# urw7rs/diffusion-models-made-easy

Hardware: AMD Instinct MI355X
Metric: denoising steps/sec + training images/sec, DDPM UNet CIFAR10 32×32 @1/2/4/8 GPU (higher is better)
Workload: dtype bf16; 1 GPU; DDPM T=1000 sampling, CIFAR10 32x32, default UNet (32,416,643 params, random init), batch 128 per GPU, t.shape=(1,); global_batch=128, parallelism=dp1 (independent chains per GPU, no data-path collective)

## Files before the change

diffusion-models-made-easy_amd/_lib.py:

```python

from __future__ import annotations

import ctypes as C
import os
import subprocess
import threading

_HERE = os.path.dirname(os.path.abspath(__file__))
LIB_PATH = os.environ.get("DMME_LIB_PATH") or os.path.join(_HERE, "libdmme_hip.so")
CSRC = os.path.join(_HERE, "csrc")

F16R32 = 4
F32, BF16, BF16X3, F16 = 0, 1, 2, 3
CHAIN_DDPM, CHAIN_DDIM, CHAIN_IDDPM, CHAIN_DDPM_GUIDED, CHAIN_DDIM_GUIDED, CHAIN_GDDIM = 0, 1, 2, 3, 4, 5
CHAIN_DDPM_CFG, CHAIN_GDDIM_CFG = 6, 7
CHAIN_DPMPP, CHAIN_DPMPP_CFG = 8, 9
CHAIN_REPAINT = 10
ARCH_DDPM, ARCH_IDDPM, ARCH_CLASSIFIER, ARCH_DDPM_COND = 0, 1, 2, 3
DTYPES = {"fp32": F32, "float32": F32, "32": F32, "bf16": BF16, "bfloat16": BF16, "16": BF16, "bf16-mixed": BF16, "16-mixed": BF16,
          "bf16x3": BF16X3, "fp16": F16, "float16": F16, "half": F16, "fp16r32": F16R32}

_lock = threading.Lock()
_lib = None

# ... 85 lines not shown
    "dmme_unet_pack_params_bwd": (_i, [_vp, _vp, _vp, _vp]),
    "dmme_unet_backward": (_i, [_vp, _vp, _vp, _vp, _vp, _i, _vp, _vp, _vp, _vp, _vp, _vp, _vp]),
    "dmme_unet_backward_buckets": (_i, [_vp, _vp, _vp, _vp, _vp, _i, _vp, _vp, _vp, _vp, _vp, _vp, _vp, BUCKET_FN, _vp]),
    "dmme_unet_backward_input": (_i, [_vp, _vp, _vp, _vp, _vp, _i, _vp, _vp, _vp, _vp, _vp, _vp]),
    "dmme_unet_plan_grad_buckets": (_i, [_vp, C.POINTER(_i64), C.POINTER(_i64), C.POINTER(_i), _i]),
    "dmme_unet_plan_bwd_summary": (_i, [_vp, C.c_char_p, _i]),
    "dmme_grad_norm": (_i, [_vp, _i64, _vp, _vp, _vp]),
    "dmme_adam_step": (_i, [_vp, _vp, _vp, _vp, _vp, _i64, _f, _f, _f, _f, _i, _vp, _f, _f, _f, _vp]),
    "dmme_amp_init": (_i, [_vp, _f, _vp]),
    "dmme_amp_scale": (_i, [_vp, _i64, _vp, _vp]),
    "dmme_adam_step_amp": (_i, [_vp, _vp, _vp, _vp, _vp, _i64, _f, _f, _f, _f, _vp, _f, _f, _f, _vp, _f, _f, _i, _vp]),
    "dmme_grad_pack_bf16": (_i, [_vp, _i64, _vp, _i64, _vp]),
    "dmme_shard_reduce_bf16": (_i, [_vp, _i, _i64, _f, _vp, _vp]),
    "dmme_grad_unpack_bf16": (_i, [_vp, _i64, _vp, _vp]),
    "dmme_unet_debug_read": (_i, [_vp, _vp, C.c_char_p, _vp, _i64, C.POINTER(_i64), _vp]),
    "dmme_unet_debug_read_grad": (_i, [_vp, _vp, C.c_char_p, _vp, _i64, C.POINTER(_i64), _vp]),
    "dmme_dropout_masks": (_i, [_vp, _u64, _u64, _vp, _vp]),
    "dmme_randn": (_i, [_vp, _i64, _u64, _u64, _vp]),
    "dmme_q_sample": (_i, [_vp, _vp, _vp, _vp, _vp, _i, _i64, _vp, _vp, _vp]),
    "dmme_ddpm_step": (_i, [_vp, _vp, _vp, _f, _f, _f, _i, _i64, _vp]),
    "dmme_ddim_step": (_i, [_vp, _vp, _f, _f, _i64, _vp]),
    "dmme_gddim_step": (_i, [_vp, _vp, _vp, _f, _f, _f, _i64, _vp]),
    "dmme_slerp": (_i, [_vp, _vp, _vp, _i, _i, _i64, _vp, _vp]),
    "dmme_chain_set": (_i, [_vp, _i64, _vp, _u64, _u64, _vp]),
    "dmme_chain_update": (_i, [_i, _vp, _vp, _vp, _vp, _vp, _i, _i64, _vp]),
    "dmme_chain_step": (_i, [_vp, _vp, _vp, _vp, _vp, _i, _vp, _vp, _vp, _vp]),
    "dmme_chain_update_gddim": (_i, [_vp, _vp, _vp, _vp, _vp, _vp, _i, _i64, _vp]),
    "dmme_log_softmax_grad": (_i, [_vp, _vp, _i, _i, _i, _f, _vp, _vp, _vp, _vp]),
    "dmme_chain_update_guided": (_i, [_i, _vp, _vp, _vp, _vp, _vp, _vp, _vp, _i, _i64, _vp]),
    "dmme_guided_chain_step": (_i, [_vp, _vp, _vp, _vp, _vp, _vp, _vp, _vp, _vp, _vp, _vp, _vp, _vp, _vp, _vp, _i, _vp, _vp, _vp, _vp]),
    "dmme_mse_loss": (_i, [_vp, _vp, _i64, _vp, _vp, _f, _vp, _vp]),
    "dmme_image_batch": (_i, [_vp, _i64, _vp, _vp, _i, _i, _i, _i, _vp, _vp]),
    "dmme_grid_tile": (_i, [_vp, _i, _i, _i, _i, _i, _i, _i, _i, _i, _i, _i, _vp, _vp]),
    "dmme_iddpm_step": (_i, [_vp, _vp, _vp, _f, _f, _f, _f, _i, _i, _i64, _vp]),
    "dmme_iddpm_loss": (_i, [_vp, _vp, _vp, _vp, _vp, _vp, _i, _i64, _f, _f, _vp, _vp, _f, _vp, _vp]),
    "dmme_iddpm_loss_rows": (_i, [_vp, _vp, _vp, _vp, _vp, _vp, _i, _vp, _i, _i64, _f, _f, _vp, _vp, _vp, _f, _vp, _vp, _vp]),
    "dmme_iddpm_prior_rows": (_i, [_vp, _i, _i64, _f, _vp, _vp]),
    "dmme_tsampler_draw": (_i, [_vp, _vp, _i, _i, _f, _u64, _u64, _i, _vp, _vp, _vp, _vp]),
    "dmme_tsampler_update": (_i, [_vp, _vp, _i, _i, _vp, _vp, _i, _vp, _vp]),
    "dmme_conv2d": (_i, [C.POINTER(ConvDesc), _vp, _vp, _vp, _vp, _vp, _vp, _vp, _vp, _vp, _vp, _i, _vp, _vp]),
    "dmme_conv2d_res": (_i, [C.POINTER(ConvDesc), _vp, _vp, _vp, _vp, _vp, _vp, _vp, _vp, _vp, _i, _i, _vp, _vp, _vp, _vp]),
    "dmme_groupnorm_scale_shift": (_i, [_i, _vp, _vp, _i, _i, _i, _i, _i, _vp, _vp, _f, _vp, _vp, _vp, _i, _vp]),
    "dmme_attention": (_i, [_i, _vp, _i, _i, _i, _vp, _i, _vp]),
    "dmme_attention_proj": (_i, [_i, _vp, _i, _i, _i, _vp, _vp, _vp, _vp, _vp, _vp, _i, _vp]),
    "dmme_attention_heads": (_i, [_i, _vp, _i, _i, _i, _i, _vp, _i, _vp]),
    "dmme_nchw_to_nhwc": (_i, [_i, _vp, _i, _i, _i, _vp, _vp]),
    "dmme_nhwc_to_nchw": (_i, [_i, _vp, _i, _i, _i, _vp, _vp]),
    "dmme_pack_weight": (_i, [_i, _vp, _i, _i, _i, _vp, _vp]),
    "dmme_event_create": (_i, [C.POINTER(_vp)]),
    "dmme_event_record": (_i, [_vp, _vp]),
    "dmme_event_elapsed_ms": (_i, [_vp, _vp, C.POINTER(_f)]),
    "dmme_event_destroy": (_i, [_vp]),
    "dmme_debug_set_stamps": (_i, [_vp]),
    "dmme_debug_mfma_valu": (_i, [_i, _i, _i, _vp, _vp]),
    "dmme_debug_issue_probe": (_i, [_i, _i, _i, _i, _i, _vp, _vp, _vp]),
    "dmme_debug_l2_stream": (_i, [_vp, _i64, _i, _i, _i, _i, _vp, _vp]),
}


def lib():
    global _lib
    if _lib is not None:
        return _lib
    with _lock:
        if _lib is not None:
            return _lib
        if not os.path.exists(LIB_PATH):
            raise DmmeError(
                f"{LIB_PATH} is missing: the HIP extension is not built. Run `python -c 'import __graft_entry__ as g; g.build()'` "
                "(or `make -C diffusion-models-made-easy_amd/csrc`). There is no CPU fallback for the product path."
            )
        h = C.CDLL(LIB_PATH)
        for name, (res, args) in PROTOTYPES.items():
            fn = getattr(h, name)
            fn.restype = res
            fn.argtypes = args
        _lib = h
    return _lib


def check(rc: int, what: str = ""):
    if rc != 0:
        msg = lib().dmme_last_error().decode("utf-8", "replace")
        if rc == -2:
            raise NotImplementedError(f"{what}: {msg}")
        if rc == -1:
            raise ValueError(f"{what}: {msg}")
        raise DmmeError(f"{what} failed (status {rc}): {msg}")


def require_gpu():
    if lib().dmme_device_count() <= 0:
        raise DmmeError("libdmme_hip.so loaded but no HIP device is visible; the denoiser path only runs on an MI355X")


def dtype_code(precision) -> int:
    key = str(precision).lower()
    if key not in DTYPES:
        raise ValueError(f"unknown precision {precision!r}; use 'fp32', 'bf16', 'fp16' / 'fp16r32' (inference) or 'bf16x3'")
    return DTYPES[key]


def csrc_sha16() -> str:
    import glob
    import hashlib

# ... 19 lines not shown
```

diffusion-models-made-easy_amd/csrc/common.h:

```cpp
#pragma once

#include <hip/hip_runtime.h>
#include <stdint.h>

#include "dmme_hip.h"

namespace dmme {

void set_error(const char* fmt, ...) __attribute__((format(printf, 1, 2)));

int debug_route(const char* key, int dflt = 0);

#define DMME_CHECK_HIP(expr)                                                                          \
    do {                                                                                              \
        hipError_t e_ = (expr);                                                                       \
        if (e_ != hipSuccess) {                                                                       \
            ::dmme::set_error("%s failed: %s (%s:%d)", #expr, hipGetErrorString(e_), __FILE__, __LINE__); \
            return DMME_ERR_HIP;                                                                      \
        }                                                                                             \
    } while (0)

#define DMME_REQUIRE(cond, code, ...)        \
    do {                                     \
        if (!(cond)) {                       \
// ... 203 lines not shown
    CONV3X3_KW,
    CONV3X3_PIPE,
};
struct ConvRoute {
    int family;
    ConvTile tile;
    int BM, BN;
    int cand;
    int GT, UA;
    int NI, ring;
    int ksplit;
    int rseg;
    int vec;
    int stat_bn;
    int stat_px;
    int stat_tiles;
};
inline ConvRoute make_route(int family, int BM = 0, int BN = 0, int vec = 0) {
    ConvRoute r{};
    r.family = family;
    r.BM = r.stat_px = BM;
    r.BN = r.stat_bn = BN;
    r.vec = vec;
    return r;
}
ConvRoute conv_route(int dtype, const ConvArgs& a);
bool conv_thin_route(int dtype, const ConvArgs& a, ConvRoute& r);
bool conv1x1_split_route(int dtype, const ConvArgs& a, ConvRoute& r);
bool conv1x1_domain(int dtype, const ConvArgs& a);
bool conv1x1_as_route(int dtype, const ConvArgs& a, ConvRoute& r);
bool conv1x1_tiled_route(int dtype, const ConvArgs& a, ConvRoute& r);
bool conv3x3_split_route(int dtype, const ConvArgs& a, ConvRoute& r);
bool conv3x3_pipe_route(int dtype, const ConvArgs& a, ConvRoute& r);
bool conv3x3_ws_route(int dtype, const ConvArgs& a, ConvRoute& r);
bool conv3x3_kw_route(int dtype, const ConvArgs& a, ConvRoute& r);
bool conv_mfma_route(int dtype, const ConvArgs& a, ConvRoute& r);
void conv_generic_route(const ConvArgs& a, ConvRoute& r);
bool conv_mfma_supported(int dtype, const ConvArgs& a);
int launch_conv_generic(int dtype, const ConvArgs& a, hipStream_t s);
const char* conv_generic_kernel_name(const ConvArgs& a);
int launch_conv_mfma(const ConvRoute& r, int dtype, const ConvArgs& a, hipStream_t s);
int launch_conv_out_thin(const ConvArgs& a, hipStream_t s);
int launch_conv1x1(const ConvRoute& r, int dtype, const ConvArgs& a, hipStream_t s);
int launch_conv1x1_as(const ConvArgs& a, hipStream_t s);
int launch_conv3x3(const ConvRoute& r, int dtype, const ConvArgs& a, hipStream_t s);
int launch_conv_kw(int dtype, const ConvArgs& a, const ConvTile& g, int NI, int ring, int BM, int ksplit, hipStream_t s);
int launch_conv(int dtype, const ConvArgs& a, hipStream_t s, int force = 0);
int launch_conv(const ConvRoute& r, int dtype, const ConvArgs& a, hipStream_t s);
void conv_label(const ConvRoute& r, int dtype, const ConvArgs& a, char* buf, int cap);
bool conv_stats_query(int dtype, const ConvArgs& a, int cg, int* tiles, int* px);
bool conv_gn_in_query(int dtype, const ConvArgs& a);
bool conv1x1_tiled_gn_in_ok(const ConvArgs& a, const ConvRoute& r);
bool conv3x3_pipe_gn_in_ok(int dtype, const ConvArgs& a, const ConvRoute& r);
int conv_gn_direct_query(int dtype, const ConvArgs& a, const int* cg, int n);
int launch_gn_finalize_parts(const float* part1, int tiles1, int cnt1, int C1, const float* part2, int tiles2, int cnt2, int C2, int N, int groups,
                             const float* gamma, const float* beta, float eps, float* scale, float* shift, float* mean_rstd, const float* t_shift,
                             const float* t_scale, int t_ld, int nt, hipStream_t s);

int launch_gn_generic(int dtype, const void* src1, const void* src2, int N, int HW, int C1, int C2, int groups,
                      const float* gamma, const float* beta, float eps, float* scale, float* shift, float* mean_rstd,
                      hipStream_t s);
bool gn_fast_supported(int dtype, int N, int HW, int C1, int C2, int groups);
size_t gn_fast_scratch_floats(int N, int HW, int C, int groups);
int launch_gn_fast(int dtype, const void* src1, const void* src2, int N, int HW, int C1, int C2, int groups,
                   const float* gamma, const float* beta, float eps, float* scale, float* shift, float* mean_rstd,
                   float* partial, hipStream_t s, void* act = nullptr, int act_silu = 0, const float* dmask = nullptr);
bool gn_small_act_supported(int dtype, int HW, int C1, int C2, int groups);

int launch_attn_generic(int dtype, const void* qkv, int N, int S, int C, void* out, hipStream_t s);
int launch_attn_heads(int dtype, const void* qkv, int N, int S, int C, int heads, void* out, hipStream_t s);
int launch_attn_heads_bwd(int dtype, const void* qkv, const void* dO, int N, int S, int C, int heads, float* P, float* dS, void* dqkv, hipStream_t s);
int launch_gn_modulate(float* scale, float* shift, const float* t_shift, const float* t_scale, int ld, int nt, int N, int C, hipStream_t s);
bool attn_x3_supported(int N, int S, int C, int heads);
int launch_attn_x3(const void* qkv, int N, int S, int C, int heads, void* out, hipStream_t s);
bool attn_mfma_supported(int dtype, int N, int S, int C);
bool attn_full_takes(int S, int D);
int launch_attn_mfma(int dtype, const void* qkv, int N, int S, int C, void* out, float* lse, hipStream_t s);
bool attn_proj_fusable(int dtype, int N, int S, int C, int gn_cg, int gn_tiles);
int launch_attn_proj(int dtype, const void* qkv, int N, int S, int C, void* ctx, float* lse, const void* w, const float* bias, const void* res, void* dst,
                     float* gn_part, int gn_tiles, int gn_cg, hipStream_t s, long long* stamps = nullptr);
bool attn_heads_mfma_supported(int dtype, int N, int S, int C, int heads);
int launch_attn_heads_mfma(int dtype, const void* qkv, int N, int S, int C, int heads, void* out, float* lse, hipStream_t s);
int launch_attn_heads_bwd_mfma(int dtype, const void* qkv, const void* O, const void* dO, const float* lse, int N, int S, int C, int heads, void* P,
                               void* dS, void* dqkv, hipStream_t s);
bool attn_bwd_mfma_supported(int dtype, int N, int S, int C);
int launch_attn_bwd_mfma(int dtype, const void* qkv, const void* O, const void* dO, const float* lse, int N, int S, int C, void* P, void* dS,
                         void* dqkv, hipStream_t s);

constexpr unsigned kFwdMarkKeep = 0x4B454550u, kFwdMarkNograd = 0x4E4F4752u;
constexpr unsigned kErrNogradBackward = 0x80000000u;
int launch_time_sinusoid(const int64_t* t, int nt, const float* freqs, int half, float* out, hipStream_t s, unsigned* mark = nullptr,
                         unsigned mark_val = 0);
int launch_linear_wave(int dtype, const float* in, int nt, int K, const void* W, const float* bias, int Nout,
                       int out_silu, float* out, hipStream_t s);
int launch_label_cond(const float* z2, int nt, const float* E, const int64_t* labels, int B, int K, int emb, float* temb, float* zsave, int* status,
                      hipStream_t s);
int launch_label_grad(const float* dz2, const int64_t* labels, int B, int K, int emb, float* dE, hipStream_t s);

int launch_nchw_to_nhwc(int dtype, const float* src, int N, int C, int HW, void* dst, hipStream_t s, const unsigned* mark = nullptr,
                        unsigned* err = nullptr);
int launch_nhwc_to_nchw(int dtype, const void* src, int N, int C, int HW, float* dst, hipStream_t s);
int launch_pack_weight(int dtype, const float* src, int Cout, int Cin, int taps, void* dst, hipStream_t s);
int launch_cast_f32_to_16(int dtype, const float* src, int64_t numel, void* dst, hipStream_t s);

struct PackItem {
    int64_t src_off;
// ... 191 lines not shown
```

diffusion-models-made-easy_amd/csrc/conv_pipe.hip:

```cpp
#include <stdio.h>

#include "conv_common.h"

namespace dmme {



template <typename T, int BM, int BN, int GT, int PIPE_UA, bool ACC3 = false>
__global__ void __launch_bounds__(256, GT == 9 ? 1 : 2) conv3x3_pipe_kernel(ConvArgs a, ConvTile g, int shTW, int shTH, int ksplit) {
    constexpr int KC = Frag<T>::KC, EPV = Frag<T>::EPV;
    constexpr int MI = BM / 64, NI = BN / 64;
    constexpr int UB = BN / 32;
    extern __shared__ __attribute__((aligned(16))) char lds[];
#define PIPE_STAMP(K) do { if (a.stamps && blockIdx.x < 2 && blockIdx.y == 0 && threadIdx.x == 0) a.stamps[blockIdx.x * 8 + (K)] = (long long)wall_clock64(); } while (0)
    PIPE_STAMP(0);
    char* ldsA = lds;
    char* ldsB = lds + (size_t)g.a_rows * ROW_DATA;
    constexpr bool DMAB_OK = sizeof(T) == 2 && GT == 3 && BN == 64;
    constexpr int B_BYTES = GT * BN * ROW_DATA;
    const bool dmab = DMAB_OK && a.dma_b;
    int cur = 0;
    float* gni_par = reinterpret_cast<float*>(ldsB + (size_t)B_BYTES * (dmab ? 2 : 1));

    const int tid = threadIdx.x, lane = tid & 63, wave = tid >> 6;
// ... 203 lines not shown
                    __syncthreads();
                    store_A(nc0);
                }
                wait_vm_all();
                __syncthreads();
                cur ^= 1;
            } else {
                __syncthreads();
                if (more) {
                    store_B();
                    if (last_grp) store_A(nc0);
                }
                __syncthreads();
            }
        }
    }

    auto pix_of = [&](int m) -> int {
        const int tx = m & mTW, ty = (m >> shTW) & mTH, tn = m >> (shTW + shTH);
        const int n = n0 + tn;
        return n < a.N ? (n * a.Hout + oy0 + ty) * a.Wout + ox0 + tx : -1;
    };
    PIPE_STAMP(3);
    if (ksplit > 1) {
        float* part = a.splitk + (int64_t)blockIdx.y * a.N * a.Hout * a.Wout * a.Cout;
#pragma unroll
        for (int ni = 0; ni < NI; ++ni) {
            const int co = co0 + wn0 + ni * 32 + r;
            if (co >= a.Cout) continue;
#pragma unroll
            for (int mi = 0; mi < MI; ++mi)
#pragma unroll
                for (int j = 0; j < 16; ++j) {
                    const int opix = pix_of(wm0 + mi * 32 + (j & 3) + 8 * (j >> 2) + 4 * h);
                    if (opix >= 0) part[(int64_t)opix * a.Cout + co] = acc[mi][ni][j];
                }
        }
        PIPE_STAMP(4);
        return;
    }
    if constexpr (BM == 64) {
        if (a.n_gno > 0) {
            const bool add_trow = a.tproj && a.nt != 1 && g.TN > 1;
            conv_epilogue_stage<T, BN, MI, NI>(a, acc, co0, wn0, r, h, wm0, n0, reinterpret_cast<float*>(lds), !add_trow);
            __syncthreads();
            conv_epilogue_store_direct<T, BN>(a, co0, n0, a.Hout * a.Wout, pix_of, reinterpret_cast<float*>(lds), add_trow);
            PIPE_STAMP(4);
            return;
        }
    }
    conv_epilogue<T, BM, BN, MI, NI>(a, acc, co0, wn0, r, h, wm0, n0, g.TN, pix_of, reinterpret_cast<float*>(lds), ty_blk * g.tiles_x + tx_blk);
    PIPE_STAMP(4);
#undef PIPE_STAMP
}

template <typename T>
__global__ void __launch_bounds__(256) conv_splitk_finish_kernel(ConvArgs a, int ksplit, int64_t total4) {
    const int C4 = a.Cout / 4, hw = a.Hout * a.Wout;
    const int64_t slice = (int64_t)a.N * hw * a.Cout;
    for (int64_t q = blockIdx.x * (int64_t)blockDim.x + threadIdx.x; q < total4; q += (int64_t)gridDim.x * blockDim.x) {
        const int64_t p = q / C4;
        const int c = (int)(q - p * C4) * 4;
        float4 v = *reinterpret_cast<const float4*>(a.splitk + p * a.Cout + c);
        for (int z = 1; z < ksplit; ++z) {
            const float4 u = *reinterpret_cast<const float4*>(a.splitk + z * slice + p * a.Cout + c);
            v.x += u.x; v.y += u.y; v.z += u.z; v.w += u.w;
        }
        float f[4] = {v.x, v.y, v.z, v.w};
        const int n = (int)(p / hw);
#pragma unroll
        for (int j = 0; j < 4; ++j) {
            float fold = a.bias ? a.bias[c + j] : 0.f;
            if (a.tproj) fold += a.tproj[(int64_t)(a.nt == 1 ? 0 : n) * a.tproj_ld + c + j];
            f[j] += fold;
            if (a.res1) f[j] += to_f(((const T*)a.res1)[p * a.Cout + c + j]);
            ((T*)a.dst)[p * a.Cout + c + j] = from_f<T>(f[j]);
        }
    }
}
static int pipe_ksplit(const ConvArgs& a, const ConvTile& g, int pick, int KC) {
    if (a.has_gni) return 1;
    const bool off = (debug_route("no_splitk") != 0);
    if (off || !a.splitk || pick != 3 || a.stride != 1 || a.gn_part || a.n_gno || a.out_silu || a.out_nchw || a.res2 || a.Cout % 4) return 1;
    const int64_t wgs = (int64_t)g.tiles_m * g.tiles_n;
    if (wgs > 128) return 1;
    int ks = (a.C1 + a.C2) / KC;
    const int room = (int)(256 / wgs);
    if (ks > room) ks = room;
    if (ks > 4) ks = 4;
    const int64_t out = (int64_t)a.N * a.Hout * a.Wout * a.Cout;
    while (ks > 1 && ks * out > a.splitk_cap) --ks;
    return ks < 1 ? 1 : ks;
}

#ifndef WS_CDMA
#define WS_CDMA 1
#endif
#ifndef WS_HYB
#define WS_HYB 0
#endif
#ifndef WS_SCHED2
#define WS_SCHED2 1
#endif
#ifndef WS_TP_UNROLL
#define WS_TP_UNROLL 9
#endif
// ... 924 lines not shown
static int launch_ws2_split(const ConvRoute& r, const ConvArgs& a, hipStream_t s) {
    const ConvTile& gw = r.tile;
    static bool attr = false;
    if (!attr) {
        int rc0 = set_lds_limit(conv3x3_ws2_kernel<11, f16, 256, 1>, 160 * 1024);
        if (rc0 == DMME_OK) rc0 = set_lds_limit(conv3x3_ws2_kernel<11, f16, 256, 2>, 160 * 1024);
        if (rc0 != DMME_OK) return rc0;
        attr = true;
    }
    const int ntiles = gw.tiles_m * gw.tiles_n;
    const dim3 wgrid((unsigned)(ntiles < 256 ? ntiles : 256));
    if (a.mix == 2)
        hipLaunchKernelGGL((conv3x3_ws2_kernel<11, f16, 256, 2>), wgrid, dim3(512), ws2_lds(a, gw), s, a, gw, ilog2(gw.TW), ilog2(gw.TH), ntiles);
    else
        hipLaunchKernelGGL((conv3x3_ws2_kernel<11, f16, 256, 1>), wgrid, dim3(512), ws2_lds(a, gw), s, a, gw, ilog2(gw.TW), ilog2(gw.TH), ntiles);
    DMME_CHECK_LAUNCH();
    return DMME_OK;
}

template <typename T>
static int launch_ws_t(const ConvRoute& r, const ConvArgs& a, hipStream_t s) {
    const ConvTile& gw = r.tile;
    static bool ws_attr = false;
    if (!ws_attr) {
        int rc0 = set_lds_limit(conv3x3_ws2_kernel<11, T, 256>, 160 * 1024);
        if (rc0 == DMME_OK) rc0 = set_lds_limit(conv3x3_ws2_kernel<7, T, 128>, 160 * 1024);
        if (rc0 == DMME_OK) rc0 = set_lds_limit(conv3x3_ws2_kernel<11, T, 256, 0, true>, 160 * 1024);
        if (rc0 == DMME_OK) rc0 = set_lds_limit(conv3x3_ws2_kernel<7, T, 128, 0, true>, 160 * 1024);
        if (rc0 == DMME_OK) rc0 = set_lds_limit(conv3x3_ws2_kernel<11, T, 256, 0, false, true>, 160 * 1024);
        if (rc0 == DMME_OK) rc0 = set_lds_limit(conv3x3_ws2_kernel<11, T, 256, 0, true, true>, 160 * 1024);
        if (rc0 != DMME_OK) return rc0;
        ws_attr = true;
    }
    const int ntiles = gw.tiles_m * gw.tiles_n;
    const dim3 wgrid((unsigned)(ntiles < 256 ? ntiles : 256));
    const bool e16 = !a.res1 && !a.res2 && !debug_route("no_ws_e16");
    if (a.r_w) {
        if (r.BM == 128)
            hipLaunchKernelGGL((conv3x3_ws2_kernel<7, T, 128, 0, true>), wgrid, dim3(512), ws2_lds(a, gw), s, a, gw, ilog2(gw.TW), ilog2(gw.TH), ntiles);
        else if (e16)
            hipLaunchKernelGGL((conv3x3_ws2_kernel<11, T, 256, 0, true, true>), wgrid, dim3(512), ws2_lds(a, gw), s, a, gw, ilog2(gw.TW), ilog2(gw.TH), ntiles);
        else
            hipLaunchKernelGGL((conv3x3_ws2_kernel<11, T, 256, 0, true>), wgrid, dim3(512), ws2_lds(a, gw), s, a, gw, ilog2(gw.TW), ilog2(gw.TH), ntiles);
    } else if (r.BM == 128)
        hipLaunchKernelGGL((conv3x3_ws2_kernel<7, T, 128>), wgrid, dim3(512), ws2_lds(a, gw), s, a, gw, ilog2(gw.TW), ilog2(gw.TH), ntiles);
    else if (e16)
        hipLaunchKernelGGL((conv3x3_ws2_kernel<11, T, 256, 0, false, true>), wgrid, dim3(512), ws2_lds(a, gw), s, a, gw, ilog2(gw.TW), ilog2(gw.TH), ntiles);
    else
        hipLaunchKernelGGL((conv3x3_ws2_kernel<11, T, 256>), wgrid, dim3(512), ws2_lds(a, gw), s, a, gw, ilog2(gw.TW), ilog2(gw.TH), ntiles);
    DMME_CHECK_LAUNCH();
    return DMME_OK;
}

template <typename T, bool ACC3 = false>
static int launch_pipe_t(const ConvRoute& r, int dtype, const ConvArgs& a, hipStream_t s) {
    const ConvTile& g = r.tile;
    const int ksplit = r.ksplit;
    const dim3 grid((unsigned)(g.tiles_m * g.tiles_n), (unsigned)ksplit);
    ConvArgs ad = a;
    bool dma = false;
    const size_t lds = pipe_launch_lds(dtype, a, r, &dma);
    ad.dma_b = dma ? 1 : 0;
    const int shTW = ilog2(g.TW), shTH = ilog2(g.TH);
    static bool attr_done[5] = {false, false, false, false, false};
    int rc = DMME_OK;
#define DMME_PIPE_CASE(IDX, BM_, BN_, GT_, UA_, LIM)                                                                          \
    case IDX:                                                                                                                 \
        if (!attr_done[IDX]) {                                                                                                \
            rc = set_lds_limit(conv3x3_pipe_kernel<T, BM_, BN_, GT_, UA_, ACC3>, (LIM) * 1024);                               \
            attr_done[IDX] = rc == DMME_OK;                                                                                   \
        }                                                                                                                     \
        if (rc == DMME_OK) hipLaunchKernelGGL((conv3x3_pipe_kernel<T, BM_, BN_, GT_, UA_, ACC3>), grid, dim3(256), lds, s, ad, g, shTW, shTH, ksplit); \
        break;
    switch (r.cand) {
        DMME_PIPE_CASE(0, 128, 128, 3, 8, 80)
        DMME_PIPE_CASE(1, 128, 64, 3, 8, 80)
        DMME_PIPE_CASE(2, 64, 64, 3, 8, 80)
        DMME_PIPE_CASE(3, 64, 64, 9, 11, 128)
        DMME_PIPE_CASE(4, 64, 64, 3, 10, 80)
    }
#undef DMME_PIPE_CASE
    if (rc != DMME_OK) return rc;
    DMME_CHECK_LAUNCH();
    if (ksplit > 1) {
        const int64_t total4 = (int64_t)a.N * a.Hout * a.Wout * (a.Cout / 4);
        hipLaunchKernelGGL(conv_splitk_finish_kernel<T>, dim3((unsigned)((total4 + 255) / 256)), dim3(256), 0, s, a, ksplit, total4);
        DMME_CHECK_LAUNCH();
    }
    return DMME_OK;
}

int launch_conv3x3(const ConvRoute& r, int dtype, const ConvArgs& a, hipStream_t s) {
    switch (r.family) {
        case CONV3X3_SPLIT: return launch_ws2_split(r, a, s);
        case CONV3X3_WS: return dtype == DMME_F16 ? launch_ws_t<f16>(r, a, s) : launch_ws_t<bf16>(r, a, s);
        case CONV3X3_KW: return launch_conv_kw(dtype, a, r.tile, r.NI, r.ring, r.BM, r.ksplit, s);
        default: break;
    }
    if (dtype == DMME_BF16) return launch_pipe_t<bf16>(r, dtype, a, s);
    if (dtype == DMME_F16) return launch_pipe_t<f16>(r, dtype, a, s);
    return a.x3 ? launch_pipe_t<float, true>(r, dtype, a, s) : launch_pipe_t<float>(r, dtype, a, s);
}

}
```

diffusion-models-made-easy_amd/csrc/plan.hip:

```cpp
#include "plan.h"

#include <functional>
#include <map>
#include <mutex>

namespace dmme {

static thread_local char g_err[512] = "";
void set_error(const char* fmt, ...) {
    va_list ap;
    va_start(ap, fmt);
    vsnprintf(g_err, sizeof(g_err), fmt, ap);
    va_end(ap);
}

int debug_route(const char* key, int dflt) {
    const char* e = getenv("DMME_DEBUG_ROUTE");
    if (!e || !*e) return dflt;
    const size_t kl = strlen(key);
    for (const char* p = e; *p;) {
        const char* end = strchr(p, ',');
        const size_t len = end ? (size_t)(end - p) : strlen(p);
        if (len >= kl && !strncmp(p, key, kl) && (len == kl || p[kl] == '=')) return len == kl ? 1 : atoi(p + kl + 1);
        if (!end) break;
// ... 1738 lines not shown
    DMME_REQUIRE(eps && target && loss && scratch, DMME_ERR_INVALID, "mse_loss: null argument");
    return launch_mse(eps, target, numel, loss, d_eps, grad_scale, scratch, (hipStream_t)stream);
}

DMME_API int dmme_debug_issue_probe(int kind, int n_inner, int iters, int flags, int blocks, void* sink, const void* src, void* stream) {
    return launch_issue_probe(kind, n_inner, iters, flags, blocks, (long long*)sink, src, (hipStream_t)stream);
}
DMME_API int dmme_debug_mfma_valu(int mode, int iters, int blocks, void* sink, void* stream) {
    DMME_REQUIRE(sink && iters > 0 && blocks > 0, DMME_ERR_INVALID, "mfma_valu: bad argument");
    return launch_mfma_valu(mode, iters, blocks, (float*)sink, (hipStream_t)stream);
}
DMME_API int dmme_debug_l2_stream(const void* buf, int64_t bytes, int iters, int mode, int depth, int blocks, void* sink, void* stream) {
    return launch_l2_stream(buf, bytes, iters, mode, depth, blocks, (unsigned*)sink, (hipStream_t)stream);
}

static long long* g_stamps = nullptr;
DMME_API int dmme_debug_set_stamps(void* buf) {
    g_stamps = (long long*)buf;
    return DMME_OK;
}

DMME_API int dmme_conv2d(const dmme_conv_desc* d, const void* src1, const void* src2, const void* weight, const float* bias,
                const float* scale, const float* shift, const float* dmask, const float* tproj, const void* res1,
                const void* res2, int R1, void* dst, void* stream) {
    DMME_REQUIRE(d && src1 && weight && bias && dst, DMME_ERR_INVALID, "conv2d: null argument");
    DMME_REQUIRE(d->taps == 9 || d->taps == 1, DMME_ERR_INVALID, "conv2d: taps must be 1 or 9");
    DMME_REQUIRE(d->stride == 1 || d->stride == 2, DMME_ERR_INVALID, "conv2d: stride must be 1 or 2");
    ConvArgs a{};
    a.src1 = src1; a.src2 = src2; a.w = weight; a.bias = bias; a.scale = scale; a.shift = shift; a.dmask = dmask;
    a.tproj = d->nt > 0 ? tproj : nullptr;
    a.res1 = res1; a.res2 = res2; a.R1 = R1; a.dst = dst;
    a.N = d->N; a.Hin = d->Hin; a.Win = d->Win; a.C1 = d->C1; a.C2 = src2 ? d->C2 : 0;
    a.up = d->upsample; a.stride = d->stride; a.taps = d->taps;
    const int Hv = a.up ? 2 * a.Hin : a.Hin, Wv = a.up ? 2 * a.Win : a.Win;
    a.Hout = Hv / a.stride; a.Wout = Wv / a.stride; a.Cout = d->Cout;
    a.pro_silu = d->pro_silu; a.out_silu = d->out_silu; a.nt = d->nt; a.tproj_ld = d->tproj_ld;
    a.in_nchw = d->in_nchw; a.out_nchw = d->out_nchw;
    a.stamps = g_stamps;
    DMME_REQUIRE(d->dtype == DMME_F32 || d->dtype == DMME_BF16 || d->dtype == DMME_BF16X3 || d->dtype == DMME_F16 || d->dtype == DMME_F16R32, DMME_ERR_INVALID,
                 "conv2d: bad dtype %d", d->dtype);
    a.x3 = d->dtype == DMME_BF16X3;
    a.f16 = d->dtype == DMME_F16;
    if (d->dtype == DMME_F16R32) {
        a.mix = a.out_nchw ? 3 : a.taps == 1 ? 4 : 1;
        a.f16 = 1;
        const ConvRoute r = conv_route(DMME_F16, a);
        DMME_REQUIRE(r.family == (a.mix == 4 ? CONV1X1_SPLIT : a.mix == 3 ? CONV_THIN : CONV3X3_SPLIT), DMME_ERR_UNSUPPORTED, "conv2d(fp16r32): the %s does not take this shape",
                     a.mix == 4 ? "split-pass 1x1 kernel" : a.mix == 3 ? "thin output conv" : "split-pass 3x3 kernel");
        return launch_conv(r, DMME_F16, a, (hipStream_t)stream);
    }
    return launch_conv(a.x3 ? DMME_F32 : d->dtype, a, (hipStream_t)stream, d->force_generic);
}

DMME_API int dmme_conv2d_res(const dmme_conv_desc* d, const void* src1, const void* src2, const void* weight, const float* bias, const float* scale,
                             const float* shift, const float* dmask, const void* r_src1, const void* r_src2, int r_C1, int r_C2, const void* r_weight,
                             const float* r_bias, void* dst, void* stream) {
    DMME_REQUIRE(d && src1 && weight && bias && dst && r_src1 && r_weight && r_bias, DMME_ERR_INVALID, "conv2d_res: null argument");
    DMME_REQUIRE(d->dtype == DMME_BF16 || d->dtype == DMME_F16, DMME_ERR_UNSUPPORTED, "conv2d_res: 16-bit tensors only (dtype %d)", d->dtype);
    ConvArgs a{};
    a.src1 = src1; a.src2 = src2; a.w = weight; a.bias = bias; a.scale = scale; a.shift = shift; a.dmask = dmask; a.dst = dst;
    a.N = d->N; a.Hin = d->Hin; a.Win = d->Win; a.C1 = d->C1; a.C2 = src2 ? d->C2 : 0;
    a.up = d->upsample; a.stride = d->stride; a.taps = d->taps;
    a.Hout = a.Hin; a.Wout = a.Win; a.Cout = d->Cout;
    a.pro_silu = d->pro_silu; a.out_silu = d->out_silu;
    a.f16 = d->dtype == DMME_F16;
    a.stamps = g_stamps;
    a.r_src1 = r_src1; a.r_src2 = r_C2 > 0 ? r_src2 : nullptr; a.r_C1 = r_C1; a.r_C2 = r_C2 > 0 ? r_C2 : 0; a.r_w = r_weight; a.r_bias = r_bias;
    const ConvRoute r = conv_route(d->dtype, a);
    DMME_REQUIRE(a.taps == 9 && a.stride == 1 && !a.up && r.rseg, DMME_ERR_UNSUPPORTED,
                 "conv2d_res: the wave-specialised 3x3 kernel does not take this shape with a residual segment (%d+%d -> %d channels, %d+%d raw, %dx%dx%d)", a.C1, a.C2,
                 a.Cout, a.r_C1, a.r_C2, a.N, a.Hin, a.Win);
    return launch_conv(r, d->dtype, a, (hipStream_t)stream);
}

DMME_API int dmme_groupnorm_scale_shift(int dtype, const void* src1, const void* src2, int N, int HW, int C1, int C2, int groups,
                               const float* gamma, const float* beta, float eps, float* scale, float* shift,
                               float* partial_scratch, int force_generic, void* stream) {
    DMME_REQUIRE(src1 && gamma && beta && scale && shift, DMME_ERR_INVALID, "groupnorm: null argument");
    if (!src2) C2 = 0;
    DMME_REQUIRE(groups > 0 && (C1 + C2) % groups == 0, DMME_ERR_INVALID, "groupnorm: %d channels not divisible by %d groups",
                 C1 + C2, groups);
    if (!force_generic && partial_scratch && gn_fast_supported(dtype, N, HW, C1, C2, groups))
        return launch_gn_fast(dtype, src1, src2, N, HW, C1, C2, groups, gamma, beta, eps, scale, shift, nullptr,
                              partial_scratch, (hipStream_t)stream);
    return launch_gn_generic(dtype, src1, src2, N, HW, C1, C2, groups, gamma, beta, eps, scale, shift, nullptr,
                             (hipStream_t)stream);
}

DMME_API int dmme_attention(int dtype, const void* qkv, int N, int S, int C, void* out, int force_generic, void* stream) {
    DMME_REQUIRE(qkv && out && N > 0 && S > 0 && C > 0, DMME_ERR_INVALID, "attention: bad argument");
    if (dtype == DMME_BF16X3) {
        if (!force_generic && attn_x3_supported(N, S, C, 1)) return launch_attn_x3(qkv, N, S, C, 1, out, (hipStream_t)stream);
        dtype = DMME_F32;
    }
    if (!force_generic && attn_mfma_supported(dtype, N, S, C)) return launch_attn_mfma(dtype, qkv, N, S, C, out, nullptr, (hipStream_t)stream);
    return launch_attn_generic(dtype, qkv, N, S, C, out, (hipStream_t)stream);
}

DMME_API int dmme_attention_proj(int dtype, const void* qkv, int N, int S, int C, const void* w, const float* bias, const void* res, void* dst, void* ctx,
                                 float* gn_part, int gn_cg, void* stream) {
    DMME_REQUIRE(qkv && w && bias && res && dst && N > 0 && S > 0 && C > 0, DMME_ERR_INVALID, "attention_proj: bad argument");
    return launch_attn_proj(dtype, qkv, N, S, C, ctx, nullptr, w, bias, res, dst, gn_part, S / 32, gn_cg, (hipStream_t)stream, g_stamps);
}

DMME_API int dmme_attention_heads(int dtype, const void* qkv, int N, int S, int C, int heads, void* out, int force_generic, void* stream) {
    DMME_REQUIRE(qkv && out && N > 0 && S > 0 && C > 0 && heads > 0 && C % heads == 0, DMME_ERR_INVALID, "attention_heads: bad argument");
// ... 45 lines not shown
```

include/dmme_hip.h:

```cpp
#ifndef DMME_HIP_H
#define DMME_HIP_H

#include <stddef.h>
#include <stdint.h>

#if defined(DMME_BUILD)
#define DMME_API __attribute__((visibility("default")))
#else
#define DMME_API
#endif

#ifdef __cplusplus
extern "C" {
#endif

typedef enum {
    DMME_OK = 0,
    DMME_ERR_INVALID = -1,
    DMME_ERR_UNSUPPORTED = -2,
    DMME_ERR_HIP = -3,
    DMME_ERR_NOMEM = -4
} dmme_status;

typedef enum { DMME_F32 = 0, DMME_BF16 = 1, DMME_BF16X3 = 2, DMME_F16 = 3, DMME_F16R32 = 4 } dmme_dtype;
// ... 188 lines not shown


DMME_API int dmme_iddpm_loss_rows(const float* model_out, const float* x_t, const float* x_0, const float* target, const int64_t* t,
                                  const float* coef, int T, const float* weight, int B, int64_t chw, float w_simple, float w_vlb, float* loss,
                                  float* rows, float* d_out, float grad_scale, int* status, float* scratch, void* stream);

DMME_API int dmme_iddpm_prior_rows(const float* x_0, int B, int64_t chw, float alpha_bar_T, float* prior, void* stream);

DMME_API int dmme_tsampler_draw(const float* hist, const int* count, int T, int H, float uniform_prob, uint64_t philox_seed,
                                uint64_t philox_offset, int B, int64_t* t, float* weight, float* p, void* stream);

DMME_API int dmme_tsampler_update(float* hist, int* count, int T, int H, const int64_t* t, const float* L, int B, int* status, void* stream);

typedef struct {
    int dtype;
    int N, Hin, Win;
    int C1, C2;
    int upsample;
    int stride;
    int taps;
    int Cout;
    int pro_silu;
    int out_silu;
    int nt;
    int tproj_ld;
    int in_nchw;
    int out_nchw;
    int force_generic;
} dmme_conv_desc;

DMME_API int dmme_conv2d(const dmme_conv_desc* d, const void* src1, const void* src2, const void* weight,
                const float* bias, const float* scale, const float* shift, const float* dmask,
                const float* tproj, const void* res1, const void* res2, int R1, void* dst, void* stream);

DMME_API int dmme_conv2d_res(const dmme_conv_desc* d, const void* src1, const void* src2, const void* weight, const float* bias,
                const float* scale, const float* shift, const float* dmask, const void* r_src1, const void* r_src2, int r_C1,
                int r_C2, const void* r_weight, const float* r_bias, void* dst, void* stream);

DMME_API int dmme_groupnorm_scale_shift(int dtype, const void* src1, const void* src2, int N, int HW, int C1, int C2,
                               int groups, const float* gamma, const float* beta, float eps, float* scale,
                               float* shift, float* partial_scratch, int force_generic, void* stream);

DMME_API int dmme_attention(int dtype, const void* qkv, int N, int S, int C, void* out, int force_generic, void* stream);
DMME_API int dmme_attention_proj(int dtype, const void* qkv, int N, int S, int C, const void* w, const float* bias, const void* res,
                                 void* dst, void* ctx, float* gn_part, int gn_cg, void* stream);

DMME_API int dmme_attention_heads(int dtype, const void* qkv, int N, int S, int C, int heads, void* out, int force_generic, void* stream);

DMME_API int dmme_nchw_to_nhwc(int dtype, const float* src, int N, int C, int HW, void* dst, void* stream);
DMME_API int dmme_nhwc_to_nchw(int dtype, const void* src, int N, int C, int HW, float* dst, void* stream);
DMME_API int dmme_pack_weight(int dtype, const float* src, int Cout, int Cin, int taps, void* dst, void* stream);

DMME_API int dmme_debug_set_stamps(void* buf);

DMME_API int dmme_event_create(void** ev);
DMME_API int dmme_event_record(void* ev, void* stream);
DMME_API int dmme_event_elapsed_ms(void* start, void* stop, float* ms);
DMME_API int dmme_event_destroy(void* ev);

#ifdef __cplusplus
}
#endif
#endif
```

Baseline: 450.9 denoising steps/s (one step = UNet forward + DDPM update on a batch of 128), summed over GPUs.

## Add persistent ring-buffered 3x3 stride-2 conv kernel with in-loop DMA interleave

Adds a new kernel for 16-bit 3x3 stride-2 downsampling convolutions. It is persistent, with the grid capped at 256 blocks, and it prefetches the next tile's halo and filter slices into LDS while the current tile computes. The global-to-LDS DMA is spread across the MFMA sequence, with explicit vmcnt waits and double-buffered halo regions, and the four waves' partial accumulators are reduced through LDS before the shared epilogue. The aim is to hide load latency and launch tail on the small downsample convs in the UNet. In exchange it uses a large LDS footprint (one block per CU), adds cross-wave reduction overhead, and is only eligible for a narrow set of shapes.

Measured after the change: 453.0 denoising steps/s (one step = UNet forward + DDPM update on a batch of 128), summed over GPUs (median of 6 runs). About the same (+0.5%).

```diff
diff --git a/diffusion-models-made-easy_amd/_lib.py b/diffusion-models-made-easy_amd/_lib.py
--- a/diffusion-models-made-easy_amd/_lib.py
+++ b/diffusion-models-made-easy_amd/_lib.py
@@ -161,6 +161,7 @@
     "dmme_event_elapsed_ms": (_i, [_vp, _vp, C.POINTER(_f)]),
     "dmme_event_destroy": (_i, [_vp]),
     "dmme_debug_set_stamps": (_i, [_vp]),
+    "dmme_debug_conv_body": (_i, [C.POINTER(ConvDesc)]),
     "dmme_debug_mfma_valu": (_i, [_i, _i, _i, _vp, _vp]),
     "dmme_debug_issue_probe": (_i, [_i, _i, _i, _i, _i, _vp, _vp, _vp]),
     "dmme_debug_l2_stream": (_i, [_vp, _i64, _i, _i, _i, _i, _vp, _vp]),
diff --git a/diffusion-models-made-easy_amd/csrc/common.h b/diffusion-models-made-easy_amd/csrc/common.h
--- a/diffusion-models-made-easy_amd/csrc/common.h
+++ b/diffusion-models-made-easy_amd/csrc/common.h
@@ -279,6 +279,7 @@
 bool conv_gn_in_query(int dtype, const ConvArgs& a);
 bool conv1x1_tiled_gn_in_ok(const ConvArgs& a, const ConvRoute& r);
 bool conv3x3_pipe_gn_in_ok(int dtype, const ConvArgs& a, const ConvRoute& r);
+int conv3x3_pipe_body(int dtype, const ConvArgs& a, const ConvRoute& r);
 int conv_gn_direct_query(int dtype, const ConvArgs& a, const int* cg, int n);
 int launch_gn_finalize_parts(const float* part1, int tiles1, int cnt1, int C1, const float* part2, int tiles2, int cnt2, int C2, int N, int groups,
                              const float* gamma, const float* beta, float eps, float* scale, float* shift, float* mean_rstd, const float* t_shift,
diff --git a/diffusion-models-made-easy_amd/csrc/conv_pipe.hip b/diffusion-models-made-easy_amd/csrc/conv_pipe.hip
--- a/diffusion-models-made-easy_amd/csrc/conv_pipe.hip
+++ b/diffusion-models-made-easy_amd/csrc/conv_pipe.hip
@@ -279,6 +279,244 @@
     conv_epilogue<T, BM, BN, MI, NI>(a, acc, co0, wn0, r, h, wm0, n0, g.TN, pix_of, reinterpret_cast<float*>(lds), ty_blk * g.tiles_x + tx_blk);
     PIPE_STAMP(4);
 #undef PIPE_STAMP
+}
+
+constexpr int S2R_PASSES = 11, S2R_PA = 6, S2R_PB = S2R_PASSES - S2R_PA;
+constexpr int S2R_HROWS = 32 * S2R_PASSES;
+constexpr int S2R_HBYTES = S2R_HROWS * ROW_DATA;
+constexpr int S2R_FBYTES = 3 * 64 * ROW_DATA;
+constexpr int S2R_OFF_F = S2R_HBYTES, S2R_OFF_H1 = S2R_HBYTES + 3 * S2R_FBYTES;
+constexpr int S2R_LDS = 2 * S2R_HBYTES + 3 * S2R_FBYTES;
+constexpr int S2R_NF = 6;
+static_assert(S2R_LDS <= 160 * 1024 && S2R_FBYTES + S2R_HBYTES >= 4 * 4 * 16 * 64 * 4 && kDirectLds <= S2R_FBYTES + S2R_HBYTES, "s2ring: LDS plan");
+struct S2Tile { int n0, oy0, ox0, co0, ts; };
+static_assert(S2R_PA + S2R_NF + S2R_PB < 64, "vmcnt is a 6-bit counter");
+
+__device__ __forceinline__ void wait_vm_all_visible() {
+#if defined(__HIP_DEVICE_COMPILE__)
+    __builtin_amdgcn_s_waitcnt(0x0F70);
+    asm volatile("" ::: "memory");
+#endif
+}
+
+template <typename T>
+__global__ void __launch_bounds__(256, 1) conv3x3_s2ring_kernel(ConvArgs a, ConvTile g, int shTW, int shTH, int ntiles) {
+    constexpr int KC = 64, EPV = 8, BM = 64, BN = 64;
+    extern __shared__ __attribute__((aligned(16))) char lds[];
+#define S2R_STAMP(K) do { if (a.stamps && blockIdx.x < 2 && threadIdx.x == 0) { a.stamps[blockIdx.x * 8 + (K)] = (long long)wall_clock64(); wait_vm_all_visible(); } } while (0)
+    S2R_STAMP(0);
+    const int tid = threadIdx.x, lane = tid & 63, wave = __builtin_amdgcn_readfirstlane(tid >> 6);
+    const int r = lane & 31, h = lane >> 5;
+    const int cu = tid & 7, urow = tid >> 3;
+    const int Cin = a.C1, nchunks = Cin / KC;
+    const int mTW = (1 << shTW) - 1, mTH = (1 << shTH) - 1;
+    const int halo_px = g.HH * g.HWd;
+    const unsigned lds0 = (unsigned)__builtin_amdgcn_readfirstlane((int)(unsigned)(size_t)(lds_c*)lds) + (unsigned)(wave * 8 * ROW_DATA);
+    const unsigned src_piece = (unsigned)((cu ^ ((urow >> 1) & 7)) * EPV);
+    const char* wbase = (const char*)a.w;
+    const char* sbase = (const char*)a.src1;
+
+    unsigned a_off[S2R_PASSES];
+    unsigned okmask = 0;
+    unsigned bd_off[2];
+    auto set_tile = [&](int t) __attribute__((always_inline)) -> S2Tile {
+        const int tile_n = t % g.tiles_n, tile_m = t / g.tiles_n;
+        const int tx_blk = tile_m % g.tiles_x, ty_blk = (tile_m / g.tiles_x) % g.tiles_y;
+        S2Tile w;
+        w.n0 = (tile_m / (g.tiles_x * g.tiles_y)) * g.TN;
+        w.oy0 = ty_blk << shTH;
+        w.ox0 = tx_blk << shTW;
+        w.co0 = tile_n * BN;
+        w.ts = ty_blk * g.tiles_x + tx_blk;
+#pragma unroll
+        for (int k = 0; k < 2; ++k) {
+            const int row = urow + 32 * k;
+            const int co = w.co0 + row < a.Cout ? w.co0 + row : a.Cout - 1;
+            bd_off[k] = ((unsigned)(co * 9 * Cin) + src_piece) * 2u;
+        }
+        okmask = 0;
+#pragma unroll
+        for (int i = 0; i < S2R_PASSES; ++i) {
+            const int row = urow + 32 * i;
+            const int tn = (int)__umulhi((unsigned)row, g.magic_px), rem = row - tn * halo_px;
+            const int hy = (int)__umulhi((unsigned)rem, g.magic_w), hx = rem - hy * g.HWd;
+            const int n = w.n0 + tn, iy = 2 * w.oy0 - 1 + hy, ix = 2 * w.ox0 - 1 + hx;
+            const bool ok = row < g.a_rows && n < a.N && iy >= 0 && iy < a.Hin && ix >= 0 && ix < a.Win;
+            const int pix = ok ? (n * a.Hin + iy) * a.Win + ix : 0;
+            a_off[i] = ((unsigned)(pix * Cin) + src_piece) * 2u;
+            okmask |= ok ? 1u << i : 0u;
+        }
+        return w;
+    };
+    auto dma_H = [&](int c0, unsigned hb, const int P0, const int P1) __attribute__((always_inline)) {
+        const char* sp = sbase + (size_t)c0 * 2;
+#pragma unroll
+        for (int i = 0; i < S2R_PASSES; ++i)
+            if (i >= P0 && i < P1) glds16_hidden_s(sp, a_off[i], hb + (unsigned)(i * 32 * ROW_DATA));
+    };
+    auto dma_F = [&](int c0, int grp, unsigned fb) __attribute__((always_inline)) {
+#pragma unroll
+        for (int j = 0; j < 3; ++j) {
+            const char* wp = wbase + ((size_t)(grp * 3 + j) * Cin + c0) * 2;
+#pragma unroll
+            for (int k = 0; k < 2; ++k) glds16_hidden_s(wp, bd_off[k], fb + (unsigned)((j * BN + 32 * k) * ROW_DATA));
+        }
+    };
+    auto dma_H1 = [&](int c0, unsigned hb, const int i) __attribute__((always_inline)) {
+        glds16_hidden_s(sbase + (size_t)c0 * 2, a_off[i], hb + (unsigned)(i * 32 * ROW_DATA));
+    };
+    auto dma_F1 = [&](int c0, int grp, unsigned fb, const int i) __attribute__((always_inline)) {
+        glds16_hidden_s(wbase + ((size_t)(grp * 3 + (i >> 1)) * Cin + c0) * 2, bd_off[i & 1], fb + (unsigned)(((i >> 1) * BN + 32 * (i & 1)) * ROW_DATA));
+    };
+    auto zero_H = [&](char* hb) __attribute__((always_inline)) {
+#pragma unroll
+        for (int i = 0; i < S2R_PASSES; ++i)
+            if (!((okmask >> i) & 1u)) *reinterpret_cast<uint4*>(hb + (urow + 32 * i) * ROW_DATA + cu * 16) = make_uint4(0u, 0u, 0u, 0u);
+    };
+    auto prime = [&]() __attribute__((always_inline)) {
+        dma_H(0, lds0, 0, S2R_PASSES);
+        dma_F(0, 0, lds0 + S2R_OFF_F);
+        dma_F(0, 1, lds0 + S2R_OFF_F + S2R_FBYTES);
+    };
+
+    int t = blockIdx.x;
+    S2Tile cur = set_tile(t);
+    prime();
+    S2R_STAMP(1);
+
+    int a_row[2], b_addr[2];
+    const int cidx = 2 * wave + h;
+#pragma unroll
+    for (int mi = 0; mi < 2; ++mi) {
+        const int m = mi * 32 + r;
+        const int tx = m & mTW, ty = (m >> shTW) & mTH, tn = m >> (shTW + shTH);
+        a_row[mi] = (tn * g.HH + 2 * ty) * g.HWd + 2 * tx;
+    }
+#pragma unroll
+    for (int ni = 0; ni < 2; ++ni) {
+        const int row = ni * 32 + r;
+        b_addr[ni] = row * ROW_DATA + ((cidx ^ ((row >> 1) & 7)) << 4);
+    }
+    char* const ldsF = lds + S2R_OFF_F;
+    float* const red = reinterpret_cast<float*>(lds + S2R_OFF_F + 2 * S2R_FBYTES);
+    bool first = true;
+
+    for (;;) {
+        wait_vm_all_visible();
+        zero_H(lds);
+        lds_barrier();
+        if (first) S2R_STAMP(2);
+
+        f32x16 acc[2][2];
+#pragma unroll
+        for (int mi = 0; mi < 2; ++mi)
+#pragma unroll
+            for (int ni = 0; ni < 2; ++ni)
+#pragma unroll
+                for (int j = 0; j < 16; ++j) acc[mi][ni][j] = 0.f;
+
+#pragma unroll 1
+        for (int ch = 0; ch < nchunks; ++ch) {
+            const bool next = ch + 1 < nchunks;
+            const int hcur = (ch & 1) ? S2R_OFF_H1 : 0, hnxt = (ch & 1) ? 0 : S2R_OFF_H1;
+#pragma unroll
+            for (int grp = 0; grp < 3; ++grp) {
+                const unsigned fb = lds0 + (unsigned)(S2R_OFF_F + ((grp + 2) % 3) * S2R_FBYTES);
+                const unsigned hnb = lds0 + (unsigned)hnxt;
+                const bool do_F = grp == 0 || next;
+                const int f_c0 = (grp == 0 ? ch : ch + 1) * KC;
+                constexpr int kP0[3] = {0, S2R_PA, 0}, kNP[3] = {S2R_PA, S2R_PB, 0};
+                const char* hb = lds + hcur;
+                const char* fbr = ldsF + grp * S2R_FBYTES;
+                uint4 af[3][2], bfr[3][2];
+                auto read_frags = [&](const int j) __attribute__((always_inline)) {
+                    const int tap_off = grp * g.HWd + j;
+#pragma unroll
+                    for (int mi = 0; mi < 2; ++mi) {
+                        const int row = a_row[mi] + tap_off;
+                        af[j][mi] = *reinterpret_cast<const uint4*>(hb + row * ROW_DATA + ((cidx ^ ((row >> 1) & 7)) << 4));
+                    }
+#pragma unroll
+                    for (int ni = 0; ni < 2; ++ni) bfr[j][ni] = *reinterpret_cast<const uint4*>(fbr + j * BN * ROW_DATA + b_addr[ni]);
+                };
+                read_frags(0);
+                read_frags(1);
+#pragma unroll
+                for (int m = 0; m < 12; ++m) {
+                    __builtin_amdgcn_sched_barrier(0);
+                    if (m < S2R_NF) {
+                        if (do_F) dma_F1(f_c0, (grp + 2) % 3, fb, m);
+                    } else if (m - S2R_NF < kNP[grp]) {
+                        if (next) dma_H1((ch + 1) * KC, hnb, kP0[grp] + m - S2R_NF);
+                    }
+                    if (m == 4) read_frags(2);
+                    __builtin_amdgcn_sched_barrier(0);
+                    mma_group(af[m >> 2][(m >> 1) & 1], bfr[m >> 2][m & 1], acc[(m >> 1) & 1][m & 1], (T*)nullptr);
+                }
+                __builtin_amdgcn_sched_barrier(0);
+                if (grp == 0) {
+                    if (next) wait_vm_keep<S2R_NF + S2R_PA>(); else wait_vm_keep<S2R_NF>();
+                } else if (grp == 1) {
+                    if (next) wait_vm_keep<S2R_PA + S2R_NF + S2R_PB>(); else wait_vm_keep<0>();
+                } else if (next) {
+                    wait_vm_keep<S2R_NF>();
+                    zero_H(lds + hnxt);
+                }
+                lds_barrier();
+            }
+        }
+        if (first) S2R_STAMP(3);
+
+        const int t_next = t + (int)gridDim.x;
+        const bool more = t_next < ntiles;
+        S2Tile nxt = cur;
+        if (more) {
+            nxt = set_tile(t_next);
+            prime();
+        }
+#pragma unroll
+        for (int mi = 0; mi < 2; ++mi)
+#pragma unroll
+            for (int ni = 0; ni < 2; ++ni) {
+                const int q = mi * 2 + ni;
+#pragma unroll
+                for (int j = 0; j < 16; ++j) red[((wave * 4 + q) * 16 + j) * 64 + lane] = acc[mi][ni][j];
+            }
+        lds_barrier();
+        f32x16 tot[1][1];
+#pragma unroll
+        for (int w = 0; w < 4; ++w) {
+            f32x16 p;
+#pragma unroll
+            for (int j = 0; j < 16; ++j) p[j] = red[((w * 4 + wave) * 16 + j) * 64 + lane];
+            if (w == 0)
+                tot[0][0] = p;
+            else
+                tot[0][0] += p;
+        }
+        lds_barrier();
+        const int wm0 = (wave >> 1) * 32, wn0 = (wave & 1) * 32;
+        const int n0 = cur.n0, oy0 = cur.oy0, ox0 = cur.ox0, co0 = cur.co0;
+        auto pix_of = [&](int m) -> int {
+            const int tx = m & mTW, ty = (m >> shTW) & mTH, tn = m >> (shTW + shTH);
+            const int n = n0 + tn;
+            return n < a.N ? (n * a.Hout + oy0 + ty) * a.Wout + ox0 + tx : -1;
+        };
+        if (a.n_gno > 0) {
+            const bool add_trow = a.tproj && a.nt != 1 && g.TN > 1;
+            conv_epilogue_stage<T, BN, 1, 1>(a, tot, co0, wn0, r, h, wm0, n0, red, !add_trow);
+            __syncthreads();
+            conv_epilogue_store_direct<T, BN>(a, co0, n0, a.Hout * a.Wout, pix_of, red, add_trow);
+        } else {
+            conv_epilogue<T, BM, BN, 1, 1>(a, tot, co0, wn0, r, h, wm0, n0, g.TN, pix_of, red, cur.ts);
+        }
+        if (!more) break;
+        cur = nxt;
+        t = t_next;
+        first = false;
+    }
+    S2R_STAMP(4);
+#undef S2R_STAMP
 }
 
 template <typename T>
@@ -1309,8 +1547,36 @@
     return DMME_OK;
 }
 
+int conv3x3_pipe_body(int dtype, const ConvArgs& a, const ConvRoute& r) {
+    if (r.family != CONV3X3_PIPE || debug_route("no_pipe_s2ring")) return 0;
+    if (!is16(dtype) || a.x3 || a.mix || a.stride != 2 || a.taps != 9 || a.up || a.in_nchw) return 0;
+    if (a.C2 || a.scale || a.dmask || a.pro_silu || a.has_gni || a.r_w) return 0;
+    if (a.C1 % 64 || r.BM != 64 || r.BN != 64 || r.ksplit != 1 || r.tile.a_rows > S2R_HROWS) return 0;
+    if ((int64_t)a.N * a.Hin * a.Win * a.C1 >= (1ll << 31) || (int64_t)a.Cout * 9 * a.C1 >= (1ll << 31)) return 0;
+    if ((int64_t)r.tile.tiles_m * r.tile.tiles_n > 2 * 256) return 0;
+    return 1;
+}
+
+template <typename T>
+static int launch_s2ring_t(const ConvRoute& r, const ConvArgs& a, hipStream_t s) {
+    const ConvTile& g = r.tile;
+    static bool attr = false;
+    if (!attr) {
+        const int rc = set_lds_limit(conv3x3_s2ring_kernel<T>, S2R_LDS);
+        if (rc != DMME_OK) return rc;
+        attr = true;
+    }
+    const int ntiles = g.tiles_m * g.tiles_n;
+    hipLaunchKernelGGL((conv3x3_s2ring_kernel<T>), dim3((unsigned)(ntiles < 256 ? ntiles : 256)), dim3(256), S2R_LDS, s, a, g, ilog2(g.TW), ilog2(g.TH), ntiles);
+    DMME_CHECK_LAUNCH();
+    return DMME_OK;
+}
+
 template <typename T, bool ACC3 = false>
 static int launch_pipe_t(const ConvRoute& r, int dtype, const ConvArgs& a, hipStream_t s) {
+    if constexpr (sizeof(T) == 2) {
+        if (conv3x3_pipe_body(dtype, a, r) == 1) return launch_s2ring_t<T>(r, a, s);
+    }
     const ConvTile& g = r.tile;
     const int ksplit = r.ksplit;
     const dim3 grid((unsigned)(g.tiles_m * g.tiles_n), (unsigned)ksplit);
diff --git a/diffusion-models-made-easy_amd/csrc/plan.hip b/diffusion-models-made-easy_amd/csrc/plan.hip
--- a/diffusion-models-made-easy_amd/csrc/plan.hip
+++ b/diffusion-models-made-easy_amd/csrc/plan.hip
@@ -1814,6 +1814,19 @@
     return launch_conv(a.x3 ? DMME_F32 : d->dtype, a, (hipStream_t)stream, d->force_generic);
 }
 
+DMME_API int dmme_debug_conv_body(const dmme_conv_desc* d) {
+    if (!d || d->force_generic || (d->dtype != DMME_BF16 && d->dtype != DMME_F16) || (d->taps != 9 && d->taps != 1) || (d->stride != 1 && d->stride != 2)) return 0;
+    ConvArgs a{};
+    a.N = d->N; a.Hin = d->Hin; a.Win = d->Win; a.C1 = d->C1; a.C2 = d->C2;
+    a.up = d->upsample; a.stride = d->stride; a.taps = d->taps;
+    const int Hv = a.up ? 2 * a.Hin : a.Hin, Wv = a.up ? 2 * a.Win : a.Win;
+    a.Hout = Hv / a.stride; a.Wout = Wv / a.stride; a.Cout = d->Cout;
+    a.pro_silu = d->pro_silu; a.out_silu = d->out_silu; a.nt = d->nt; a.tproj_ld = d->tproj_ld;
+    a.in_nchw = d->in_nchw; a.out_nchw = d->out_nchw;
+    a.f16 = d->dtype == DMME_F16;
+    return conv3x3_pipe_body(d->dtype, a, conv_route(d->dtype, a));
+}
+
 DMME_API int dmme_conv2d_res(const dmme_conv_desc* d, const void* src1, const void* src2, const void* weight, const float* bias, const float* scale,
                              const float* shift, const float* dmask, const void* r_src1, const void* r_src2, int r_C1, int r_C2, const void* r_weight,
                              const float* r_bias, void* dst, void* stream) {
diff --git a/include/dmme_hip.h b/include/dmme_hip.h
--- a/include/dmme_hip.h
+++ b/include/dmme_hip.h
@@ -264,6 +264,7 @@
 DMME_API int dmme_pack_weight(int dtype, const float* src, int Cout, int Cin, int taps, void* dst, void* stream);
 
 DMME_API int dmme_debug_set_stamps(void* buf);
+DMME_API int dmme_debug_conv_body(const dmme_conv_desc* d);
 
 DMME_API int dmme_event_create(void** ev);
 DMME_API int dmme_event_record(void* ev, void* stream);
```
